# tomvanbraeckel/amv-codec-tools

Measured on AMD Instinct MI355X. Metric: AMV frames/sec/GPU (160x120 decode, bit-exact), higher is better.
Workload: dtype int32; 1 GPU; 160x120 AMV decode, 160000-frame synthetic stream per GPU, chunks resident in HBM; parallelism=frame-range x1, frames_per_gpu=160000, stream=seeded synthetic source (BASELINE.md section 4), every frame

## Files before the change

### amv-codec-tools_amd/csrc/amv_block_load.h

```cpp
#pragma once
#include <cstdlib>

#include "amv_kernels.h"
#include "amv_piece_map.h"

namespace amv {

constexpr uint32_t kSegImageBytes = 60u * 128u;
constexpr uint32_t kScatterSwizzleMask = 0x38u;
constexpr uint32_t kScatterFieldShift = 6u;
constexpr uint32_t kScatterAddressMask = 0x11ffeu;

__device__ __forceinline__ void seg_sync() {
    __builtin_amdgcn_fence(__ATOMIC_SEQ_CST, "wavefront");
    __builtin_amdgcn_wave_barrier();
}

__device__ __forceinline__ bool select_frame(const FrameSel& sel, uint32_t n, uint32_t item, uint32_t& f, uint32_t& slot) {
    f = slot = item;
    if (!sel.round) return true;
    const uint32_t p = sel.base + item;
    if (item >= sel.round || p >= (sel.count ? *sel.count : n)) return false;
    f = sel.list ? sel.list[p] : p;
    return true;
}

struct Segment {
    uint32_t f, slot;
    uint32_t m0, cnt, ok, mcu0;
    uint32_t segidx, nsegs;
};
__device__ __forceinline__ Segment segment_of(uint32_t f, uint32_t slot, const uint32_t* __restrict__ nmcu_ok, const FrameGeom& g,
                                              uint32_t nseg, uint32_t my, uint32_t seg) {
    const uint32_t m0 = seg * kSegMcus;
    return {f, slot, m0, min(kSegMcus, g.mcu_cols - m0), nmcu_ok[f], my * g.mcu_cols + m0, my * nseg + seg, g.mcu_rows * nseg};
}
template <bool kRound>
__device__ __forceinline__ bool next_item(const PieceMap& pm, uint32_t& item) {
    if (!kRound) return false;
    seg_sync();
    item += piece_stride(pm);
    return true;
}

__device__ __forceinline__ bool load_segment_blocks(const SyncSinks& in, const Segment& sg, bool dense_only, const FrameGeom& g,
                                                    uint32_t lane, uint8_t* s_img, uint32_t (&c)[32], bool& skip) {
    const uint32_t f = sg.f, slot = sg.slot, segidx = sg.segidx, nsegs = sg.nsegs, mcu0 = sg.mcu0, cnt = sg.cnt, ok = sg.ok;
    const uint32_t nb = cnt * 6u;
    uint32_t rc = 0xffffffffu, r0 = 0u, r1 = 0u;
    if (in.rec != nullptr && !dense_only) {
        const uint32_t* ss = in.seg_start + ((uint64_t)f * (nsegs + 1u) + segidx) * 2u;
        rc = in.rec_count[f];
        r0 = ss[0];
        r1 = ss[3];
    }
    const bool records = rc != 0xffffffffu;
    skip = !records && in.rec != nullptr && !dense_only;
    if (skip) return false;
    int dc_base = 0;
    if (records) {
        const uint32_t ok_blocks = in.ok_in_blocks ? ok : ok * 6u;
        const uint32_t blocks_ok_here = ok_blocks > mcu0 * 6u ? min(nb, ok_blocks - mcu0 * 6u) : 0u;
        if (!blocks_ok_here) r1 = r0;
        struct __attribute__((packed, aligned(4))) Rec4 { uint32_t w[4]; };
        constexpr uint32_t kAhead = 3;
        const uint32_t* rec = in.rec + (uint64_t)in.rec_line[f] * 32u + r0;
        const uint32_t nrec = r1 - r0;
        Rec4 q[kAhead];
#pragma unroll
        for (uint32_t j = 0; j < kAhead; ++j) {
            const uint32_t i = j * 4u * kWave + lane * 4u;
            q[j] = Rec4{{kDummyRecord, kDummyRecord, kDummyRecord, kDummyRecord}};
            if (i < nrec) q[j] = *reinterpret_cast<const Rec4*>(rec + i);
        }
        uint4* img16 = reinterpret_cast<uint4*>(s_img);
        if (nb == 60u) {
            constexpr uint32_t kWhole = 60u * 8u / kWave;
#pragma unroll
            for (uint32_t j = 0; j < kWhole; ++j) img16[j * kWave + lane] = make_uint4(0, 0, 0, 0);
            if (lane < 60u * 8u - kWhole * kWave) img16[kWhole * kWave + lane] = make_uint4(0, 0, 0, 0);
        } else {
            for (uint32_t i = lane; i < nb * 8u; i += kWave) img16[i] = make_uint4(0, 0, 0, 0);
        }
        seg_sync();
        const uint32_t field0 = (mcu0 * 6u - g.blocks) & 63u;
        const uint32_t first6 = (uint32_t)__builtin_amdgcn_readfirstlane((int)((64u - field0) << kScatterFieldShift));
        const uint32_t ok7 = blocks_ok_here << 7;
        const uint32_t spare = kSegImageBytes + lane * 2u;
        for (uint32_t base = 0;;) {
#pragma unroll
            for (uint32_t j = 0; j < kAhead; ++j) {
                if (base + j * 4u * kWave >= nrec) break;
                if (base + (j + 1u) * 4u * kWave > nrec) {
                    const int32_t left = (int32_t)(nrec - base - j * 4u * kWave) - (int32_t)(lane * 4u);
#pragma unroll
                    for (uint32_t e = 0; e < 4u; ++e)
                        if (left <= (int32_t)e) q[j].w[e] = kDummyRecord;
                }
#pragma unroll
                for (uint32_t e = 0; e < 4u; ++e) {
                    const uint32_t w = q[j].w[e];
                    uint32_t t;
                    asm("v_add_lshl_u32 %0, %1, %2, 1" : "=v"(t) : "v"(w ^ ((w >> 3) & kScatterSwizzleMask)), "s"(first6));
                    const uint32_t at = t & kScatterAddressMask;
                    *reinterpret_cast<int16_t*>(s_img + (at < ok7 ? at : spare)) = (int16_t)(w >> 16);
                }
            }
            base += kAhead * 4u * kWave;
            if (base >= nrec) break;
#pragma unroll
            for (uint32_t j = 0; j < kAhead; ++j) {
                const uint32_t i = base + j * 4u * kWave + lane * 4u;
                if (i < nrec) q[j] = *reinterpret_cast<const Rec4*>(rec + i);
            }
        }
        const uint32_t frame_lanes = ((rc >> 24) & 63u) + 1u;
        if (frame_lanes > 1u) {
            const uint32_t babs = mcu0 * 6u + lane, k6 = lane % 6u;
            const uint4 ent = lane < frame_lanes ? reinterpret_cast<const uint4*>(in.lane_tab)[(uint64_t)f * in.lanes + lane]
                                                 : make_uint4(0xffffffffu, 0u, 0u, 0u);
            uint32_t at = 0u;
#pragma unroll
            for (uint32_t step = 32u; step >= 1u; step >>= 1) {
                const uint32_t probe = at + step;
                const uint32_t first = (uint32_t)__shfl((int)ent.x, (int)(probe & 63u));
                if (probe < frame_lanes && first <= babs) at = probe;
            }
            const int by = __shfl((int)ent.y, (int)at), bu = __shfl((int)ent.z, (int)at), bv = __shfl((int)ent.w, (int)at);
            dc_base = at ? (k6 < 4u ? by : (k6 == 4u ? bu : bv)) : 0;
        }
        seg_sync();
    }
    if (lane >= nb) return false;
    if (records) {
        const uint4* src = reinterpret_cast<const uint4*>(s_img) + lane * 8u;
        const uint32_t swz = (lane + mcu0 * 6u - g.blocks) & 7u;
#pragma unroll
        for (int i = 0; i < 8; ++i) {
            const uint4 q = src[(uint32_t)i ^ swz];
            c[4 * i] = q.x; c[4 * i + 1] = q.y; c[4 * i + 2] = q.z; c[4 * i + 3] = q.w;
        }
        c[0] = (c[0] & 0xffff0000u) | ((c[0] + (uint32_t)dc_base) & 0xffffu);
    } else {
        const uint4* src = reinterpret_cast<const uint4*>(in.coef + (((uint64_t)slot * g.mcus + mcu0) * 6u + lane) * 64u);
#pragma unroll
        for (int i = 0; i < 8; ++i) {
            const uint4 q = src[i];
            c[4 * i] = q.x; c[4 * i + 1] = q.y; c[4 * i + 2] = q.z; c[4 * i + 3] = q.w;
        }
    }
    return true;
}

__device__ __forceinline__ int coef_at(const uint32_t (&c)[32], int i) {
    return (i & 1) ? ((int)c[i >> 1] >> 16) : (int)(int16_t)(c[i >> 1] & 0xffffu);
}

template <class Kernel, class... Tail>
static inline void launch_segments(Kernel part, Kernel walk, uint32_t block, uint32_t row_groups, const SyncSinks& sinks, const uint32_t* nmcu_ok,
                            uint32_t n, const FrameSel& sel, uint32_t items, const FrameGeom& g, hipStream_t s, Tail... tail) {
    for_each_launch(row_groups, segs_per_row(g), items, sel.round != 0u, [&](const PieceMap& pm, uint32_t grid) {
        hipLaunchKernelGGL(sel.round ? walk : part, dim3(grid), dim3(block), 0, s, sinks, nmcu_ok, n, sel, g, pm, tail...);
    });
}

}
```

### amv-codec-tools_amd/csrc/amv_piece_map.h

```cpp
#pragma once
#include <cstdint>
#include <cstdlib>

#include "amv_segment.h"

namespace amv {

struct PieceMap {
    uint32_t row_groups, magic_rg;
    uint32_t nseg, magic_8ns;
    uint32_t units;
    uint32_t item_base;
};
AMV_HD inline uint32_t mul_hi(uint32_t a, uint32_t b) { return (uint32_t)(((uint64_t)a * b) >> 32); }
AMV_HD inline uint32_t div_by(uint32_t b, uint32_t d, uint32_t magic) { return d == 1u ? b : mul_hi(b, magic); }

AMV_HD inline bool locate_piece(const PieceMap& pm, uint32_t b, uint32_t& item0, uint32_t& row_group, uint32_t& seg) {
    const uint32_t octet = pm.nseg == 1u ? b >> 3 : mul_hi(b, pm.magic_8ns);
    const uint32_t within = b - octet * 8u * pm.nseg;
    const uint32_t unit = octet * 8u + (within & 7u);
    seg = within >> 3;
    const uint32_t local = div_by(unit, pm.row_groups, pm.magic_rg);
    row_group = unit - local * pm.row_groups;
    item0 = pm.item_base + local;
    return unit < pm.units;
}
AMV_HD inline uint32_t piece_stride(const PieceMap& pm) { return pm.units / pm.row_groups; }

inline PieceMap make_piece_map(uint32_t row_groups, uint32_t nseg) {
    auto magic = [](uint32_t d) { return (uint32_t)((0x100000000ull + d - 1u) / d); };
    return PieceMap{row_groups, magic(row_groups), nseg, magic(8u * nseg), 0u, 0u};
}
inline uint32_t set_walkers(PieceMap& pm, uint32_t walkers) {
    pm.units = walkers * pm.row_groups;
    return (pm.units + 7u) / 8u * 8u * pm.nseg;
}
inline uint32_t most_items(const PieceMap& pm) {
    const uint32_t widest = 8u * pm.nseg > pm.row_groups ? 8u * pm.nseg : pm.row_groups;
    const uint32_t most = (0xffffffffu / widest - 8u * pm.nseg) / (pm.row_groups * pm.nseg);
    if (const char* e = getenv("AMVHIP_RECON_MOST")) {
        const long v = atol(e);
        if (v > 0 && (unsigned long)v < most) return (uint32_t)v;
    }
    return most;
}

template <class Launch>
static inline void for_each_launch(uint32_t row_groups, uint32_t nseg, uint32_t items, bool round, Launch launch, uint32_t most = 0u) {
    PieceMap pm = make_piece_map(row_groups, nseg);
    if (round) {
        const uint32_t grid = set_walkers(pm, items < kRoundWalkers ? items : kRoundWalkers);
        if (items) launch(pm, grid);
        return;
    }
    if (!most) most = most_items(pm);
    for (uint32_t base = 0; base < items; base += most) {
        pm.item_base = base;
        const uint32_t grid = set_walkers(pm, items - base < most ? items - base : most);
        launch(pm, grid);
    }
}

}
```

### amv-codec-tools_amd/csrc/amv_reconstruct.hip

```cpp
#include "amv_block_load.h"

namespace amv {

namespace {

struct __attribute__((aligned(4))) Px12 { uint32_t w[3]; };

constexpr int kRowsPerGroup = 4;

__device__ __forceinline__ int mad24(int x, int w, int c) {
    int d;
    asm("v_mad_i32_i24 %0, %1, %2, %3" : "=v"(d) : "v"(x), "s"(w), "v"(c));
    return d;
}

enum RowKind { kRowPlain, kRow0, kRow4 };

constexpr uint32_t inverse_of_odd(uint32_t a) {
    uint32_t x = a;
    for (int i = 0; i < 5; ++i) x *= 2u - a * x;
    return x;
}
constexpr int kRowSeed = (int)((64u * inverse_of_odd(181u)) & 0x7fffffffu);
static_assert(181u * 2u * (uint32_t)kRowSeed == 128u, "the seed puts 128 into both 181-products");

template <bool kColumn, RowKind kKind = kRowPlain>
__device__ __forceinline__ void idct8(int& v0, int& v1, int& v2, int& v3, int& v4, int& v5, int& v6, int& v7) {
    constexpr int W1 = 2841, W2 = 2676, W3 = 2408, W5 = 1609, W6 = 1108, W7 = 565;
    constexpr int kBias = kKind == kRow0 ? 128 + 8192 : 128;
    constexpr int kRound = kColumn ? 4 : 0;
    constexpr int kDown = kColumn ? 3 : 0;
    constexpr int kOut = kColumn ? 7 : 8;
    constexpr int kSeed = kColumn ? 0 : kRowSeed, kHalf = kColumn ? 128 : 0;
    int a0 = kColumn ? v0 : v0 * 2048 + kBias, a1 = kColumn ? v4 : v4 * 2048;
    const int i2 = v6, i3 = v2, i4 = v1, i5 = v7, i6 = v5, i7 = v3;
    int t;
    int a4 = mad24(i4, W1, mad24(i5, W7, kRound + kSeed)) >> kDown;
    int a5 = mad24(i4, W7, mad24(i5, -W1, kRound)) >> kDown;
    int a6 = mad24(i6, W5, mad24(i7, W3, kRound - kSeed)) >> kDown;
    int a7 = mad24(i6, W3, mad24(i7, -W5, kRound)) >> kDown;
    t = a0 + a1;
    a0 -= a1;
    int a2 = mad24(i3, W6, mad24(i2, -W2, kRound)) >> kDown;
    int a3 = mad24(i3, W2, mad24(i2, W6, kRound)) >> kDown;
    a1 = a4 + a6;
    a4 -= a6;
    a6 = a5 + a7;
    a5 -= a7;
    a7 = t + a3;
    t -= a3;
    a3 = a0 + a2;
    a0 -= a2;
    a2 = (181 * (a4 + a5) + kHalf) >> 8;
    a4 = (181 * (a4 - a5) + kHalf) >> 8;
    v0 = a7 + a1;
    v1 = a3 + a2;
    v2 = a0 + a4;
    v3 = t + a6;
    v4 = t - a6;
    v5 = a0 - a4;
    v6 = a3 - a2;
    v7 = a7 - a1;
    if (kKind == kRowPlain) {
        v0 >>= kOut; v1 >>= kOut; v2 >>= kOut; v3 >>= kOut; v4 >>= kOut; v5 >>= kOut; v6 >>= kOut; v7 >>= kOut;
    } else {
        v0 &= ~255; v1 &= ~255; v2 &= ~255; v3 &= ~255; v4 &= ~255; v5 &= ~255; v6 &= ~255; v7 &= ~255;
    }
}

struct QuantWords { uint32_t w[2][16]; };
constexpr QuantWords pack_quant() {
    QuantWords q{};
    for (int i = 0; i < 64; ++i) {
        q.w[0][i >> 2] |= (uint32_t)kQuantLuma[i] << (8 * (i & 3));
        q.w[1][i >> 2] |= (uint32_t)kQuantChroma[i] << (8 * (i & 3));
    }
    return q;
}
__device__ const QuantWords kQuantWords = pack_quant();

__device__ __forceinline__ uint32_t clamp_pack(int lo, int hi) {
    uint32_t p, d;
    asm("v_cvt_pk_i16_i32 %0, %1, %2" : "=v"(p) : "v"(lo), "v"(hi));
    asm("v_pk_ashrrev_i16 %0, %1, %2" : "=v"(d) : "s"(0x00070007u), "v"(p));
    return d;
}

constexpr uint32_t pair16(int lo, int hi) { return ((uint32_t)lo & 0xffffu) | ((uint32_t)hi << 16); }
__device__ __forceinline__ uint32_t dot2_bias(uint32_t a, uint32_t w) {
    uint32_t d;
    asm("v_dot2_i32_i16 %0, %1, %2, %3" : "=v"(d) : "v"(a), "s"(w), "v"(32768u));
    return d;
}

struct ChromaTerms { uint32_t bg[2], rb[2], gr[2]; };
__device__ __forceinline__ ChromaTerms chroma_terms(uint32_t uu, uint32_t vv) {
    ChromaTerms c;
#pragma unroll
    for (int e = 0; e < 2; ++e) {
        const uint32_t uv = __builtin_amdgcn_perm(vv, uu, e ? 0x07060302u : 0x05040100u);
        const uint32_t r = dot2_bias(uv, pair16(18, 367));
        const uint32_t gg = dot2_bias(uv, pair16(-159, -220));
        const uint32_t b = dot2_bias(uv, pair16(411, -29));
        c.bg[e] = __builtin_amdgcn_perm(gg, b, 0x06050201u);
        c.rb[e] = __builtin_amdgcn_perm(b, r, 0x06050201u);
        c.gr[e] = __builtin_amdgcn_perm(r, gg, 0x06050201u);
    }
    return c;
}
template <int kLo, int kHi>
__device__ __forceinline__ uint32_t pair_sum(uint32_t yy, uint32_t cc) {
    uint32_t sum;
    if (kLo == 0 && kHi == 0) asm("v_pk_add_i16 %0, %1, %2 op_sel_hi:[0,1]" : "=v"(sum) : "v"(yy), "v"(cc));
    else if (kLo == 0 && kHi == 1) asm("v_pk_add_i16 %0, %1, %2" : "=v"(sum) : "v"(yy), "v"(cc));
    else asm("v_pk_add_i16 %0, %1, %2 op_sel:[1,0]" : "=v"(sum) : "v"(yy), "v"(cc));
    static_assert(kLo <= kHi, "(hi, lo) is not a bracket of the row");
    return sum;
}
__device__ __forceinline__ uint32_t sat_quad(uint32_t lo, uint32_t hi) {
    uint32_t d;
    asm("v_sat_pk_u8_i16 %0, %1" : "=v"(d) : "v"(lo));
    asm("v_sat_pk_u8_i16_sdwa %0, %1 dst_sel:WORD_1 dst_unused:UNUSED_PRESERVE src0_sel:DWORD" : "+v"(d) : "v"(hi));
    return d;
}
__device__ __forceinline__ Px12 patch_row(uint2 yy, const ChromaTerms& c) {
    Px12 v;
    v.w[0] = sat_quad(pair_sum<0, 0>(yy.x, c.bg[0]), pair_sum<0, 1>(yy.x, c.rb[0]));
    v.w[1] = sat_quad(pair_sum<1, 1>(yy.x, c.gr[0]), pair_sum<0, 0>(yy.y, c.bg[1]));
    v.w[2] = sat_quad(pair_sum<0, 1>(yy.y, c.rb[1]), pair_sum<1, 1>(yy.y, c.gr[1]));
    return v;
}

}

template <bool kRound, int kRows>
__global__ __launch_bounds__(kWave * kRows) void amv_reconstruct_kernel(
    SyncSinks in, const uint32_t* __restrict__ nmcu_ok, uint32_t n, FrameSel sel,
    FrameGeom g, PieceMap pm, uint32_t flags, uint8_t* __restrict__ out) {
    constexpr uint32_t kPitchY = kSegMcus * 16, kPitchC = kSegMcus * 8;
    __shared__ __attribute__((aligned(16))) int16_t s_all[kRows][16 * kPitchY + 2 * 8 * kPitchC + 64];
    static_assert((16 * kPitchY + 2 * 8 * kPitchC) * 2 == kSegImageBytes, "the planes reuse the image");
    const uint32_t lane = threadIdx.x & 63u, wave = (uint32_t)__builtin_amdgcn_readfirstlane((int)(threadIdx.x >> 6));
    uint32_t item, row_group, seg;
    if (!locate_piece(pm, blockIdx.x, item, row_group, seg)) return;
    const uint32_t my = row_group * kRows + wave;
    if (my >= g.mcu_rows) return;
    int16_t* const s_mem = s_all[wave];
    int16_t* const s_y = s_mem;
    int16_t* const s_u = s_mem + 16 * kPitchY;
    int16_t* const s_v = s_u + 8 * kPitchC;
    uint8_t* const s_img = reinterpret_cast<uint8_t*>(s_mem);

    uint32_t qw[16];
    {
        const uint4* q4 = reinterpret_cast<const uint4*>(kQuantWords.w[lane % 6u >= 4u ? 1 : 0]);
#pragma unroll
        for (int i = 0; i < 4; ++i) {
            const uint4 q = q4[i];
            qw[4 * i] = q.x; qw[4 * i + 1] = q.y; qw[4 * i + 2] = q.z; qw[4 * i + 3] = q.w;
        }
    }
    do {
    uint32_t f, slot;
    if (!select_frame(sel, n, item, f, slot)) return;
    const Segment sg = segment_of(f, slot, nmcu_ok, g, pm.nseg, my, seg);
    const uint32_t m0 = sg.m0, cnt = sg.cnt, ok = sg.ok, mcu0 = sg.mcu0;

    uint32_t c[32];
    bool skip;
    if (load_segment_blocks(in, sg, kRound, g, lane, s_img, c, skip)) {
        const uint32_t m = lane / 6u, k6 = lane % 6u;
        const bool chroma = k6 >= 4u;
        int v[64];
#pragma unroll
        for (int nat = 0; nat < 64; ++nat) {
            const int scan = kScanOfNatural[nat];
            v[nat] = coef_at(c, scan) * (int)((qw[scan >> 2] >> (8 * (scan & 3))) & 255u);
        }
        if (!(flags & kFlagZigzagFixed))
            v[kAmvlibQuirkNatural] = coef_at(c, kAmvlibQuirkScan) * (int)((qw[kAmvlibQuirkScan >> 2] >> (8 * (kAmvlibQuirkScan & 3))) & 255u);
#pragma unroll
        for (int r = 0; r < 8; ++r) {
            if (r == 0) idct8<false, kRow0>(v[0], v[1], v[2], v[3], v[4], v[5], v[6], v[7]);
            else if (r == 4) idct8<false, kRow4>(v[32], v[33], v[34], v[35], v[36], v[37], v[38], v[39]);
            else idct8<false>(v[8 * r], v[8 * r + 1], v[8 * r + 2], v[8 * r + 3], v[8 * r + 4], v[8 * r + 5], v[8 * r + 6], v[8 * r + 7]);
        }
#pragma unroll
        for (int col = 0; col < 8; ++col)
            idct8<true>(v[col], v[8 + col], v[16 + col], v[24 + col], v[32 + col], v[40 + col], v[48 + col], v[56 + col]);
        int16_t* dst = chroma ? (k6 == 4u ? s_u : s_v) + m * 8u
                              : s_y + ((k6 >> 1) * 8u) * kPitchY + m * 16u + (k6 & 1u) * 8u;
        const uint32_t pitch = chroma ? kPitchC : kPitchY;
#pragma unroll
        for (int r = 0; r < 8; ++r) {
            uint32_t w[4];
#pragma unroll
            for (int q = 0; q < 4; ++q) w[q] = clamp_pack(v[8 * r + 2 * q], v[8 * r + 2 * q + 1]);
            *reinterpret_cast<uint4*>(dst + r * pitch) = make_uint4(w[0], w[1], w[2], w[3]);
        }
    }
    if (skip) return;
    seg_sync();

    const uint32_t vr = min(16u, g.height - my * 16u);
    const uint32_t px = min(cnt * 16u, g.width - m0 * 16u);
    const uint32_t groups = cnt * 4u;
    const bool all_decoded = mcu0 + cnt <= ok;
    uint8_t* const frame = out + (uint64_t)f * g.frame_bytes;
    const uint32_t row0 = (g.height - 1u - my * 16u) * g.stride + m0 * 48u;
    constexpr uint32_t kPairY = 4u * kPitchY, kPairC = 2u * kPitchC, kPlaneU = 32u * kPitchY, kPlaneV = kPlaneU + 16u * kPitchC;
    if (all_decoded && cnt == kSegMcus && px == kSegMcus * 16u && vr == 16u) {
        constexpr uint32_t kGroups = kSegMcus * 4u, kTrips = kGroups * 8u / kWave;
        static_assert(kGroups * 8u % kWave == 0u && kGroups < kWave && kPairC == kGroups * 4u, "whole trips; chroma is linear in t");
        const uint32_t a = lane >= kGroups ? 1u : 0u, b = lane - a * kGroups;
        const uint8_t* const ly = s_img + a * kPairY + b * 8u;
        const uint8_t* const ly_past = ly + (kPairY - kGroups * 8u);
        const uint8_t* const lc = s_img + kPlaneU + lane * 4u;
        const uint32_t off0 = row0 - a * 2u * g.stride + b * 12u;
        const uint32_t off0_past = off0 - 2u * g.stride - kGroups * 12u;
#pragma unroll
        for (uint32_t k = 0; k < kTrips; ++k) {
            const uint32_t q = k * kWave / kGroups, r = k * kWave % kGroups;
            const bool past = r != 0u && b >= kGroups - r;
            const uint8_t* const y = (past ? ly_past : ly) + (q * kPairY + r * 8u);
            const uint2 ya = *reinterpret_cast<const uint2*>(y);
            const uint2 yb = *reinterpret_cast<const uint2*>(y + 2u * kPitchY);
            const uint32_t uu = *reinterpret_cast<const uint32_t*>(lc + k * kWave * 4u);
            const uint32_t vv = *reinterpret_cast<const uint32_t*>(lc + k * kWave * 4u + (kPlaneV - kPlaneU));
            const ChromaTerms c = chroma_terms(uu, vv);
            uint8_t* const upper = frame + (int64_t)(int32_t)(r * 12u - q * 2u * g.stride);
            const uint32_t off = past ? off0_past : off0;
            *reinterpret_cast<Px12*>(upper + off) = patch_row(ya, c);
            *reinterpret_cast<Px12*>(upper - g.stride + off) = patch_row(yb, c);
        }
        continue;
    }
    const uint32_t pairs = (vr + 1u) >> 1;
    const uint32_t step_i2 = kWave / groups, step_gi = kWave - step_i2 * groups;
    uint32_t i2 = lane / groups, gi = lane - i2 * groups;
    for (; i2 < pairs; i2 += step_i2, gi += step_gi) {
        if (gi >= groups) { gi -= groups; ++i2; if (i2 >= pairs) break; }
        const uint32_t lc = gi * 4u;
        uint2 ya = *reinterpret_cast<const uint2*>(s_y + (2u * i2) * kPitchY + lc);
        uint2 yb = *reinterpret_cast<const uint2*>(s_y + (2u * i2 + 1u) * kPitchY + lc);
        uint32_t uu = *reinterpret_cast<const uint32_t*>(s_u + i2 * kPitchC + (lc >> 1));
        uint32_t vv = *reinterpret_cast<const uint32_t*>(s_v + i2 * kPitchC + (lc >> 1));
        if (!all_decoded && (mcu0 + (gi >> 2)) >= ok) {
            constexpr uint32_t kDark = 0xfc00fc00u;
            ya.x = ya.y = yb.x = yb.y = kDark;
            uu = vv = 0u;
        }
        const ChromaTerms c = chroma_terms(uu, vv);
        if (lc >= px) continue;
        uint32_t off = row0 - 2u * i2 * g.stride + lc * 3u;
#pragma unroll
        for (int row = 0; row < 2; ++row) {
            const Px12 v = patch_row(row ? yb : ya, c);
            if (2u * i2 + (uint32_t)row >= vr) break;
            if (lc + 4u <= px) {
                *reinterpret_cast<Px12*>(frame + off) = v;
            } else {
#pragma unroll
                for (uint32_t q = 0; q < 9u; ++q)
                    if (q < (px - lc) * 3u) frame[off + q] = (uint8_t)(v.w[q >> 2] >> (8u * (q & 3u)));
            }
            off -= g.stride;
        }
    }
    } while (next_item<kRound>(pm, item));
}

template <int kRows, class... Args>
static void launch_rows(const FrameGeom& g, Args... args) {
    launch_segments(amv_reconstruct_kernel<false, kRows>, amv_reconstruct_kernel<true, kRows>, kWave * kRows, (g.mcu_rows + kRows - 1) / kRows, args...);
}

void launch_reconstruct(const SyncSinks& sinks, const uint32_t* nmcu_ok, uint32_t n, const FrameSel& sel, uint32_t items,
                        const FrameGeom& g, uint32_t flags, uint8_t* out, hipStream_t s) {
    const uint32_t slots4 = (g.mcu_rows + 3u) / 4u * 4u, slots5 = (g.mcu_rows + 4u) / 5u * 5u;
    const uint32_t waste4 = slots4 - g.mcu_rows, waste5 = slots5 - g.mcu_rows;
    if (10u * waste4 * slots5 >= 10u * waste5 * slots4 + slots4 * slots5) launch_rows<5>(g, sinks, nmcu_ok, n, sel, items, g, s, flags, out);
    else launch_rows<kRowsPerGroup>(g, sinks, nmcu_ok, n, sel, items, g, s, flags, out);
}

__global__ __launch_bounds__(kWave * 4) void amv_expand_records_kernel(SyncSinks in, const uint32_t* __restrict__ nmcu_ok, uint32_t n,
                                                                        FrameGeom g, uint32_t nseg, int16_t* __restrict__ coef) {
    __shared__ __attribute__((aligned(16))) uint8_t s_img[4][kSegImageBytes + 128];
    const uint32_t lane = threadIdx.x & 63u, wave = threadIdx.x >> 6;
    const uint32_t segs = g.mcu_rows * nseg;
    const uint64_t pairs = (uint64_t)n * segs;
    for (uint64_t p = (uint64_t)blockIdx.x * 4u + wave; p < pairs; p += (uint64_t)gridDim.x * 4u) {
        const uint32_t f = (uint32_t)(p / segs), segidx = (uint32_t)(p % segs);
        const Segment sg = segment_of(f, f, nmcu_ok, g, nseg, segidx / nseg, segidx % nseg);
        uint32_t c[32];
        bool skip;
        if (load_segment_blocks(in, sg, false, g, lane, s_img[wave], c, skip)) {
            const uint32_t blk = sg.mcu0 * 6u + lane;
            if (blk >= (in.ok_in_blocks ? sg.ok : sg.ok * 6u)) {
#pragma unroll
                for (int i = 0; i < 32; ++i) c[i] = 0u;
            }
            uint4* d = reinterpret_cast<uint4*>(coef + ((uint64_t)f * g.blocks + blk) * 64u);
#pragma unroll
            for (int i = 0; i < 8; ++i) d[i] = make_uint4(c[4 * i], c[4 * i + 1], c[4 * i + 2], c[4 * i + 3]);
        }
        seg_sync();
    }
}

void launch_expand_records(const SyncSinks& sinks, const uint32_t* nmcu_ok, uint32_t n, const FrameGeom& g, int16_t* coef,
                           hipStream_t s) {
    const uint32_t nseg = segs_per_row(g);
    const uint64_t groups = ((uint64_t)n * g.mcu_rows * nseg + 3u) / 4u;
    if (groups == 0) return;
    hipLaunchKernelGGL(amv_expand_records_kernel, dim3(groups < 65536u ? (uint32_t)groups : 65536u), dim3(kWave * 4), 0, s, sinks,
                       nmcu_ok, n, g, nseg, coef);
}

}
```

Baseline: 31.01 million frames/s.

## Split reconstruct into flat full-row kernel and packed half-row kernel

For 160x120 frames the last MCU row is only 8 pixels tall, so a wave assigned to it left much of its work idle. The reconstruct launch now handles full MCU rows of all frames through a flattened row list, with no per-frame row-group padding. A second kernel packs the short last rows of several frames (a frame and a half per wave) so more lanes carry blocks. The cost is an extra kernel launch and more complex lane-to-block mapping and fallback paths.

```diff
diff --git a/amv-codec-tools_amd/csrc/amv_block_load.h b/amv-codec-tools_amd/csrc/amv_block_load.h
--- a/amv-codec-tools_amd/csrc/amv_block_load.h
+++ b/amv-codec-tools_amd/csrc/amv_block_load.h
@@ -43,8 +43,8 @@
     return true;
 }
 
-__device__ __forceinline__ bool load_segment_blocks(const SyncSinks& in, const Segment& sg, bool dense_only, const FrameGeom& g,
-                                                    uint32_t lane, uint8_t* s_img, uint32_t (&c)[32], bool& skip) {
+__device__ __forceinline__ bool load_segment_blocks_at(const SyncSinks& in, const Segment& sg, bool dense_only, const FrameGeom& g,
+                                                       uint32_t lane, uint32_t blk, uint8_t* s_img, uint32_t (&c)[32], bool& skip) {
     const uint32_t f = sg.f, slot = sg.slot, segidx = sg.segidx, nsegs = sg.nsegs, mcu0 = sg.mcu0, cnt = sg.cnt, ok = sg.ok;
     const uint32_t nb = cnt * 6u;
     uint32_t rc = 0xffffffffu, r0 = 0u, r1 = 0u;
@@ -116,7 +116,7 @@
         }
         const uint32_t frame_lanes = ((rc >> 24) & 63u) + 1u;
         if (frame_lanes > 1u) {
-            const uint32_t babs = mcu0 * 6u + lane, k6 = lane % 6u;
+            const uint32_t babs = mcu0 * 6u + blk, k6 = blk % 6u;
             const uint4 ent = lane < frame_lanes ? reinterpret_cast<const uint4*>(in.lane_tab)[(uint64_t)f * in.lanes + lane]
                                                  : make_uint4(0xffffffffu, 0u, 0u, 0u);
             uint32_t at = 0u;
@@ -131,10 +131,10 @@
         }
         seg_sync();
     }
-    if (lane >= nb) return false;
+    if (blk >= nb) return false;
     if (records) {
-        const uint4* src = reinterpret_cast<const uint4*>(s_img) + lane * 8u;
-        const uint32_t swz = (lane + mcu0 * 6u - g.blocks) & 7u;
+        const uint4* src = reinterpret_cast<const uint4*>(s_img) + blk * 8u;
+        const uint32_t swz = (blk + mcu0 * 6u - g.blocks) & 7u;
 #pragma unroll
         for (int i = 0; i < 8; ++i) {
             const uint4 q = src[(uint32_t)i ^ swz];
@@ -142,7 +142,7 @@
         }
         c[0] = (c[0] & 0xffff0000u) | ((c[0] + (uint32_t)dc_base) & 0xffffu);
     } else {
-        const uint4* src = reinterpret_cast<const uint4*>(in.coef + (((uint64_t)slot * g.mcus + mcu0) * 6u + lane) * 64u);
+        const uint4* src = reinterpret_cast<const uint4*>(in.coef + (((uint64_t)slot * g.mcus + mcu0) * 6u + blk) * 64u);
 #pragma unroll
         for (int i = 0; i < 8; ++i) {
             const uint4 q = src[i];
@@ -150,6 +150,10 @@
         }
     }
     return true;
+}
+__device__ __forceinline__ bool load_segment_blocks(const SyncSinks& in, const Segment& sg, bool dense_only, const FrameGeom& g,
+                                                    uint32_t lane, uint8_t* s_img, uint32_t (&c)[32], bool& skip) {
+    return load_segment_blocks_at(in, sg, dense_only, g, lane, lane, s_img, c, skip);
 }
 
 __device__ __forceinline__ int coef_at(const uint32_t (&c)[32], int i) {
diff --git a/amv-codec-tools_amd/csrc/amv_piece_map.h b/amv-codec-tools_amd/csrc/amv_piece_map.h
--- a/amv-codec-tools_amd/csrc/amv_piece_map.h
+++ b/amv-codec-tools_amd/csrc/amv_piece_map.h
@@ -61,4 +61,56 @@
     }
 }
 
+
+struct RowList {
+    uint32_t rows_full, magic, total;
+};
+inline RowList make_row_list(uint32_t n, uint32_t rows_full) {
+    return RowList{rows_full, rows_full ? (uint32_t)((0x100000000ull + rows_full - 1u) / rows_full) : 0u, n * rows_full};
 }
+AMV_HD inline void flat_row(const RowList& rl, uint32_t r, uint32_t& f, uint32_t& my) {
+    f = div_by(r, rl.rows_full, rl.magic);
+    my = r - f * rl.rows_full;
+}
+
+struct HalfRowPart {
+    uint32_t f, m0, cnt;
+};
+struct HalfRowPlan {
+    uint32_t n, mcu_cols, nseg, magic_ns;
+    uint32_t pack3;
+    uint32_t waves;
+};
+inline HalfRowPlan half_row_plan(uint32_t n, const FrameGeom& g) {
+    HalfRowPlan p;
+    p.n = n;
+    p.mcu_cols = g.mcu_cols;
+    p.nseg = segs_per_row(g);
+    p.magic_ns = (uint32_t)((0x100000000ull + p.nseg - 1u) / p.nseg);
+    p.pack3 = !(g.mcu_cols & 1u) && 6u * g.mcu_cols <= (uint32_t)kWave ? 1u : 0u;
+    p.waves = p.pack3 ? n / 3u * 2u + (n % 3u ? (n % 3u == 1u ? 1u : 2u) : 0u) : n * p.nseg;
+    return p;
+}
+AMV_HD inline void half_row_wave(const HalfRowPlan& p, uint32_t w, HalfRowPart& a, HalfRowPart& b) {
+    if (!p.pack3) {
+        const uint32_t f = div_by(w, p.nseg, p.magic_ns), m0 = (w - f * p.nseg) * kSegMcus;
+        a = HalfRowPart{f, m0, p.mcu_cols - m0 < kSegMcus ? p.mcu_cols - m0 : kSegMcus};
+        b = HalfRowPart{0u, 0u, 0u};
+        return;
+    }
+    const uint32_t f0 = (w >> 1) * 3u, half = p.mcu_cols >> 1;
+    if (!(w & 1u)) {
+        a = HalfRowPart{f0, 0u, p.mcu_cols};
+        b = HalfRowPart{f0 + 1u, 0u, f0 + 1u < p.n ? half : 0u};
+    } else {
+        a = HalfRowPart{f0 + 1u, half, half};
+        b = HalfRowPart{f0 + 2u, 0u, f0 + 2u < p.n ? p.mcu_cols : 0u};
+    }
+}
+inline bool split_rows_ok(uint32_t n, const FrameGeom& g) {
+    const uint32_t last = g.height & 15u, rows_full = g.mcu_rows - 1u, nseg = segs_per_row(g);
+    if (last < 1u || last > 8u || n == 0u) return false;
+    return ((uint64_t)n * rows_full + 4u) * (rows_full ? rows_full : 1u) < 0x100000000ull && ((uint64_t)n * nseg + 4u) * nseg < 0x100000000ull;
+}
+
+}
diff --git a/amv-codec-tools_amd/csrc/amv_reconstruct.hip b/amv-codec-tools_amd/csrc/amv_reconstruct.hip
--- a/amv-codec-tools_amd/csrc/amv_reconstruct.hip
+++ b/amv-codec-tools_amd/csrc/amv_reconstruct.hip
@@ -131,110 +131,40 @@
     return v;
 }
 
-}
-
-template <bool kRound, int kRows>
-__global__ __launch_bounds__(kWave * kRows) void amv_reconstruct_kernel(
-    SyncSinks in, const uint32_t* __restrict__ nmcu_ok, uint32_t n, FrameSel sel,
-    FrameGeom g, PieceMap pm, uint32_t flags, uint8_t* __restrict__ out) {
-    constexpr uint32_t kPitchY = kSegMcus * 16, kPitchC = kSegMcus * 8;
-    __shared__ __attribute__((aligned(16))) int16_t s_all[kRows][16 * kPitchY + 2 * 8 * kPitchC + 64];
-    static_assert((16 * kPitchY + 2 * 8 * kPitchC) * 2 == kSegImageBytes, "the planes reuse the image");
-    const uint32_t lane = threadIdx.x & 63u, wave = (uint32_t)__builtin_amdgcn_readfirstlane((int)(threadIdx.x >> 6));
-    uint32_t item, row_group, seg;
-    if (!locate_piece(pm, blockIdx.x, item, row_group, seg)) return;
-    const uint32_t my = row_group * kRows + wave;
-    if (my >= g.mcu_rows) return;
-    int16_t* const s_mem = s_all[wave];
-    int16_t* const s_y = s_mem;
-    int16_t* const s_u = s_mem + 16 * kPitchY;
-    int16_t* const s_v = s_u + 8 * kPitchC;
-    uint8_t* const s_img = reinterpret_cast<uint8_t*>(s_mem);
-
-    uint32_t qw[16];
-    {
-        const uint4* q4 = reinterpret_cast<const uint4*>(kQuantWords.w[lane % 6u >= 4u ? 1 : 0]);
-#pragma unroll
-        for (int i = 0; i < 4; ++i) {
-            const uint4 q = q4[i];
-            qw[4 * i] = q.x; qw[4 * i + 1] = q.y; qw[4 * i + 2] = q.z; qw[4 * i + 3] = q.w;
-        }
-    }
-    do {
-    uint32_t f, slot;
-    if (!select_frame(sel, n, item, f, slot)) return;
-    const Segment sg = segment_of(f, slot, nmcu_ok, g, pm.nseg, my, seg);
-    const uint32_t m0 = sg.m0, cnt = sg.cnt, ok = sg.ok, mcu0 = sg.mcu0;
-
-    uint32_t c[32];
-    bool skip;
-    if (load_segment_blocks(in, sg, kRound, g, lane, s_img, c, skip)) {
-        const uint32_t m = lane / 6u, k6 = lane % 6u;
-        const bool chroma = k6 >= 4u;
-        int v[64];
-#pragma unroll
-        for (int nat = 0; nat < 64; ++nat) {
-            const int scan = kScanOfNatural[nat];
-            v[nat] = coef_at(c, scan) * (int)((qw[scan >> 2] >> (8 * (scan & 3))) & 255u);
-        }
-        if (!(flags & kFlagZigzagFixed))
-            v[kAmvlibQuirkNatural] = coef_at(c, kAmvlibQuirkScan) * (int)((qw[kAmvlibQuirkScan >> 2] >> (8 * (kAmvlibQuirkScan & 3))) & 255u);
-#pragma unroll
-        for (int r = 0; r < 8; ++r) {
-            if (r == 0) idct8<false, kRow0>(v[0], v[1], v[2], v[3], v[4], v[5], v[6], v[7]);
-            else if (r == 4) idct8<false, kRow4>(v[32], v[33], v[34], v[35], v[36], v[37], v[38], v[39]);
-            else idct8<false>(v[8 * r], v[8 * r + 1], v[8 * r + 2], v[8 * r + 3], v[8 * r + 4], v[8 * r + 5], v[8 * r + 6], v[8 * r + 7]);
-        }
-#pragma unroll
-        for (int col = 0; col < 8; ++col)
-            idct8<true>(v[col], v[8 + col], v[16 + col], v[24 + col], v[32 + col], v[40 + col], v[48 + col], v[56 + col]);
-        int16_t* dst = chroma ? (k6 == 4u ? s_u : s_v) + m * 8u
-                              : s_y + ((k6 >> 1) * 8u) * kPitchY + m * 16u + (k6 & 1u) * 8u;
-        const uint32_t pitch = chroma ? kPitchC : kPitchY;
-#pragma unroll
-        for (int r = 0; r < 8; ++r) {
-            uint32_t w[4];
-#pragma unroll
-            for (int q = 0; q < 4; ++q) w[q] = clamp_pack(v[8 * r + 2 * q], v[8 * r + 2 * q + 1]);
-            *reinterpret_cast<uint4*>(dst + r * pitch) = make_uint4(w[0], w[1], w[2], w[3]);
-        }
-    }
-    if (skip) return;
-    seg_sync();
-
-    const uint32_t vr = min(16u, g.height - my * 16u);
-    const uint32_t px = min(cnt * 16u, g.width - m0 * 16u);
+__device__ __forceinline__ void load_quant(bool chroma, uint32_t (&qw)[16]) {
+    const uint4* q4 = reinterpret_cast<const uint4*>(kQuantWords.w[chroma ? 1 : 0]);
+#pragma unroll
+    for (int i = 0; i < 4; ++i) {
+        const uint4 q = q4[i];
+        qw[4 * i] = q.x; qw[4 * i + 1] = q.y; qw[4 * i + 2] = q.z; qw[4 * i + 3] = q.w;
+    }
+}
+
+__device__ __forceinline__ void transform_block(const uint32_t (&c)[32], const uint32_t (&qw)[16], uint32_t flags, int (&v)[64]) {
+#pragma unroll
+    for (int nat = 0; nat < 64; ++nat) {
+        const int scan = kScanOfNatural[nat];
+        v[nat] = coef_at(c, scan) * (int)((qw[scan >> 2] >> (8 * (scan & 3))) & 255u);
+    }
+    if (!(flags & kFlagZigzagFixed))
+        v[kAmvlibQuirkNatural] = coef_at(c, kAmvlibQuirkScan) * (int)((qw[kAmvlibQuirkScan >> 2] >> (8 * (kAmvlibQuirkScan & 3))) & 255u);
+#pragma unroll
+    for (int r = 0; r < 8; ++r) {
+        if (r == 0) idct8<false, kRow0>(v[0], v[1], v[2], v[3], v[4], v[5], v[6], v[7]);
+        else if (r == 4) idct8<false, kRow4>(v[32], v[33], v[34], v[35], v[36], v[37], v[38], v[39]);
+        else idct8<false>(v[8 * r], v[8 * r + 1], v[8 * r + 2], v[8 * r + 3], v[8 * r + 4], v[8 * r + 5], v[8 * r + 6], v[8 * r + 7]);
+    }
+#pragma unroll
+    for (int col = 0; col < 8; ++col)
+        idct8<true>(v[col], v[8 + col], v[16 + col], v[24 + col], v[32 + col], v[40 + col], v[48 + col], v[56 + col]);
+}
+
+template <uint32_t kPitchY, uint32_t kPitchC>
+__device__ __forceinline__ void store_patches(const int16_t* s_y, const int16_t* s_u, const int16_t* s_v, uint32_t lane, uint8_t* frame,
+                                              uint32_t row0, uint32_t stride, uint32_t vr, uint32_t px, uint32_t cnt, uint32_t mcu0,
+                                              uint32_t ok) {
     const uint32_t groups = cnt * 4u;
     const bool all_decoded = mcu0 + cnt <= ok;
-    uint8_t* const frame = out + (uint64_t)f * g.frame_bytes;
-    const uint32_t row0 = (g.height - 1u - my * 16u) * g.stride + m0 * 48u;
-    constexpr uint32_t kPairY = 4u * kPitchY, kPairC = 2u * kPitchC, kPlaneU = 32u * kPitchY, kPlaneV = kPlaneU + 16u * kPitchC;
-    if (all_decoded && cnt == kSegMcus && px == kSegMcus * 16u && vr == 16u) {
-        constexpr uint32_t kGroups = kSegMcus * 4u, kTrips = kGroups * 8u / kWave;
-        static_assert(kGroups * 8u % kWave == 0u && kGroups < kWave && kPairC == kGroups * 4u, "whole trips; chroma is linear in t");
-        const uint32_t a = lane >= kGroups ? 1u : 0u, b = lane - a * kGroups;
-        const uint8_t* const ly = s_img + a * kPairY + b * 8u;
-        const uint8_t* const ly_past = ly + (kPairY - kGroups * 8u);
-        const uint8_t* const lc = s_img + kPlaneU + lane * 4u;
-        const uint32_t off0 = row0 - a * 2u * g.stride + b * 12u;
-        const uint32_t off0_past = off0 - 2u * g.stride - kGroups * 12u;
-#pragma unroll
-        for (uint32_t k = 0; k < kTrips; ++k) {
-            const uint32_t q = k * kWave / kGroups, r = k * kWave % kGroups;
-            const bool past = r != 0u && b >= kGroups - r;
-            const uint8_t* const y = (past ? ly_past : ly) + (q * kPairY + r * 8u);
-            const uint2 ya = *reinterpret_cast<const uint2*>(y);
-            const uint2 yb = *reinterpret_cast<const uint2*>(y + 2u * kPitchY);
-            const uint32_t uu = *reinterpret_cast<const uint32_t*>(lc + k * kWave * 4u);
-            const uint32_t vv = *reinterpret_cast<const uint32_t*>(lc + k * kWave * 4u + (kPlaneV - kPlaneU));
-            const ChromaTerms c = chroma_terms(uu, vv);
-            uint8_t* const upper = frame + (int64_t)(int32_t)(r * 12u - q * 2u * g.stride);
-            const uint32_t off = past ? off0_past : off0;
-            *reinterpret_cast<Px12*>(upper + off) = patch_row(ya, c);
-            *reinterpret_cast<Px12*>(upper - g.stride + off) = patch_row(yb, c);
-        }
-        continue;
-    }
     const uint32_t pairs = (vr + 1u) >> 1;
     const uint32_t step_i2 = kWave / groups, step_gi = kWave - step_i2 * groups;
     uint32_t i2 = lane / groups, gi = lane - i2 * groups;
@@ -252,7 +182,7 @@
         }
         const ChromaTerms c = chroma_terms(uu, vv);
         if (lc >= px) continue;
-        uint32_t off = row0 - 2u * i2 * g.stride + lc * 3u;
+        uint32_t off = row0 - 2u * i2 * stride + lc * 3u;
 #pragma unroll
         for (int row = 0; row < 2; ++row) {
             const Px12 v = patch_row(row ? yb : ya, c);
@@ -264,19 +194,211 @@
                 for (uint32_t q = 0; q < 9u; ++q)
                     if (q < (px - lc) * 3u) frame[off + q] = (uint8_t)(v.w[q >> 2] >> (8u * (q & 3u)));
             }
-            off -= g.stride;
-        }
-    }
+            off -= stride;
+        }
+    }
+}
+
+}
+
+template <bool kRound, int kRows, bool kFlat = false>
+__global__ __launch_bounds__(kWave * kRows) void amv_reconstruct_kernel(
+    SyncSinks in, const uint32_t* __restrict__ nmcu_ok, uint32_t n, FrameSel sel,
+    FrameGeom g, PieceMap pm, uint32_t flags, uint8_t* __restrict__ out, RowList rl) {
+    static_assert(!(kRound && kFlat), "a round takes its frames whole");
+    constexpr uint32_t kPitchY = kSegMcus * 16, kPitchC = kSegMcus * 8;
+    __shared__ __attribute__((aligned(16))) int16_t s_all[kRows][16 * kPitchY + 2 * 8 * kPitchC + 64];
+    static_assert((16 * kPitchY + 2 * 8 * kPitchC) * 2 == kSegImageBytes, "the planes reuse the image");
+    const uint32_t lane = threadIdx.x & 63u, wave = (uint32_t)__builtin_amdgcn_readfirstlane((int)(threadIdx.x >> 6));
+    uint32_t item, row_group, seg;
+    if (!locate_piece(pm, blockIdx.x, item, row_group, seg)) return;
+    uint32_t my = row_group * kRows + wave, flat_f = 0u;
+    if (kFlat) {
+        const uint32_t r = item * kRows + wave;
+        if (r >= rl.total) return;
+        flat_row(rl, r, flat_f, my);
+    } else if (my >= g.mcu_rows) return;
+    int16_t* const s_mem = s_all[wave];
+    int16_t* const s_y = s_mem;
+    int16_t* const s_u = s_mem + 16 * kPitchY;
+    int16_t* const s_v = s_u + 8 * kPitchC;
+    uint8_t* const s_img = reinterpret_cast<uint8_t*>(s_mem);
+
+    uint32_t qw[16];
+    load_quant(lane % 6u >= 4u, qw);
+    do {
+    uint32_t f, slot;
+    if (kFlat) f = slot = flat_f;
+    else if (!select_frame(sel, n, item, f, slot)) return;
+    const Segment sg = segment_of(f, slot, nmcu_ok, g, pm.nseg, my, seg);
+    const uint32_t m0 = sg.m0, cnt = sg.cnt, ok = sg.ok, mcu0 = sg.mcu0;
+
+    uint32_t c[32];
+    bool skip;
+    if (load_segment_blocks(in, sg, kRound, g, lane, s_img, c, skip)) {
+        const uint32_t m = lane / 6u, k6 = lane % 6u;
+        const bool chroma = k6 >= 4u;
+        int v[64];
+        transform_block(c, qw, flags, v);
+        int16_t* dst = chroma ? (k6 == 4u ? s_u : s_v) + m * 8u
+                              : s_y + ((k6 >> 1) * 8u) * kPitchY + m * 16u + (k6 & 1u) * 8u;
+        const uint32_t pitch = chroma ? kPitchC : kPitchY;
+#pragma unroll
+        for (int r = 0; r < 8; ++r) {
+            uint32_t w[4];
+#pragma unroll
+            for (int q = 0; q < 4; ++q) w[q] = clamp_pack(v[8 * r + 2 * q], v[8 * r + 2 * q + 1]);
+            *reinterpret_cast<uint4*>(dst + r * pitch) = make_uint4(w[0], w[1], w[2], w[3]);
+        }
+    }
+    if (skip) return;
+    seg_sync();
+
+    const uint32_t vr = min(16u, g.height - my * 16u);
+    const uint32_t px = min(cnt * 16u, g.width - m0 * 16u);
+    const bool all_decoded = mcu0 + cnt <= ok;
+    uint8_t* const frame = out + (uint64_t)f * g.frame_bytes;
+    const uint32_t row0 = (g.height - 1u - my * 16u) * g.stride + m0 * 48u;
+    constexpr uint32_t kPairY = 4u * kPitchY, kPairC = 2u * kPitchC, kPlaneU = 32u * kPitchY, kPlaneV = kPlaneU + 16u * kPitchC;
+    if (all_decoded && cnt == kSegMcus && px == kSegMcus * 16u && vr == 16u) {
+        constexpr uint32_t kGroups = kSegMcus * 4u, kTrips = kGroups * 8u / kWave;
+        static_assert(kGroups * 8u % kWave == 0u && kGroups < kWave && kPairC == kGroups * 4u, "whole trips; chroma is linear in t");
+        const uint32_t a = lane >= kGroups ? 1u : 0u, b = lane - a * kGroups;
+        const uint8_t* const ly = s_img + a * kPairY + b * 8u;
+        const uint8_t* const ly_past = ly + (kPairY - kGroups * 8u);
+        const uint8_t* const lc = s_img + kPlaneU + lane * 4u;
+        const uint32_t off0 = row0 - a * 2u * g.stride + b * 12u;
+        const uint32_t off0_past = off0 - 2u * g.stride - kGroups * 12u;
+#pragma unroll
+        for (uint32_t k = 0; k < kTrips; ++k) {
+            const uint32_t q = k * kWave / kGroups, r = k * kWave % kGroups;
+            const bool past = r != 0u && b >= kGroups - r;
+            const uint8_t* const y = (past ? ly_past : ly) + (q * kPairY + r * 8u);
+            const uint2 ya = *reinterpret_cast<const uint2*>(y);
+            const uint2 yb = *reinterpret_cast<const uint2*>(y + 2u * kPitchY);
+            const uint32_t uu = *reinterpret_cast<const uint32_t*>(lc + k * kWave * 4u);
+            const uint32_t vv = *reinterpret_cast<const uint32_t*>(lc + k * kWave * 4u + (kPlaneV - kPlaneU));
+            const ChromaTerms c = chroma_terms(uu, vv);
+            uint8_t* const upper = frame + (int64_t)(int32_t)(r * 12u - q * 2u * g.stride);
+            const uint32_t off = past ? off0_past : off0;
+            *reinterpret_cast<Px12*>(upper + off) = patch_row(ya, c);
+            *reinterpret_cast<Px12*>(upper - g.stride + off) = patch_row(yb, c);
+        }
+        continue;
+    }
+    store_patches<kPitchY, kPitchC>(s_y, s_u, s_v, lane, frame, row0, g.stride, vr, px, cnt, mcu0, ok);
     } while (next_item<kRound>(pm, item));
+}
+
+__global__ __launch_bounds__(kWave * kRowsPerGroup) void amv_reconstruct_half_rows_kernel(
+    SyncSinks in, const uint32_t* __restrict__ nmcu_ok, HalfRowPlan hp, FrameGeom g, uint32_t flags, uint8_t* __restrict__ out) {
+    constexpr uint32_t kMcus = 15, kPitchY = kMcus * 16, kPitchC = kMcus * 8;
+    __shared__ __attribute__((aligned(16))) int16_t s_all[kRowsPerGroup][8 * kPitchY + 2 * 8 * kPitchC + 64];
+    static_assert((8 * kPitchY + 2 * 8 * kPitchC) * 2 == kSegImageBytes, "the planes reuse the image");
+    static_assert(kMcus * 4u <= (uint32_t)kWave && kMcus >= kSegMcus + kSegMcus / 2u, "a frame and a half, a lane per block that shows");
+    const uint32_t lane = threadIdx.x & 63u, wave = (uint32_t)__builtin_amdgcn_readfirstlane((int)(threadIdx.x >> 6));
+    const uint32_t w = blockIdx.x * kRowsPerGroup + wave;
+    if (w >= hp.waves) return;
+    HalfRowPart part[2];
+    half_row_wave(hp, w, part[0], part[1]);
+    int16_t* const s_mem = s_all[wave];
+    int16_t* const s_y = s_mem;
+    int16_t* const s_u = s_mem + 8 * kPitchY;
+    int16_t* const s_v = s_u + 8 * kPitchC;
+    uint8_t* const s_img = reinterpret_cast<uint8_t*>(s_mem);
+
+    const uint32_t split = part[0].cnt * 4u;
+    const bool second = lane >= split;
+    const uint32_t j = lane & 3u;
+    const uint32_t blk = ((lane - (second ? split : 0u)) >> 2) * 6u + (j < 2u ? j : j + 2u);
+    const bool chroma = j >= 2u;
+    uint32_t qw[16];
+    load_quant(chroma, qw);
+
+    const uint32_t my = g.mcu_rows - 1u, nseg = hp.nseg;
+    uint32_t okp[2] = {0u, 0u};
+    bool skip[2] = {true, true};
+    uint32_t c[32];
+    bool have = false;
+#pragma unroll
+    for (int p = 0; p < 2; ++p) {
+        if (part[p].cnt == 0u) continue;
+        const uint32_t f = part[p].f, m0 = part[p].m0;
+        okp[p] = nmcu_ok[f];
+        const Segment sg{f, f, m0, part[p].cnt, okp[p], my * g.mcu_cols + m0, my * nseg + m0 / kSegMcus, g.mcu_rows * nseg};
+        if (load_segment_blocks_at(in, sg, false, g, lane, second == (p == 1) ? blk : 0xffffffffu, s_img, c, skip[p])) have = true;
+        seg_sync();
+    }
+    if (have) {
+        int v[64];
+        transform_block(c, qw, flags, v);
+        const uint32_t m = lane >> 2;
+        int16_t* dst = chroma ? (j == 2u ? s_u : s_v) + m * 8u : s_y + m * 16u + j * 8u;
+        const uint32_t pitch = chroma ? kPitchC : kPitchY;
+#pragma unroll
+        for (int r = 0; r < 8; ++r) {
+            uint32_t q[4];
+#pragma unroll
+            for (int e = 0; e < 4; ++e) q[e] = clamp_pack(v[8 * r + 2 * e], v[8 * r + 2 * e + 1]);
+            *reinterpret_cast<uint4*>(dst + r * pitch) = make_uint4(q[0], q[1], q[2], q[3]);
+        }
+    }
+    seg_sync();
+    const uint32_t vr = g.height - my * 16u;
+    const uint32_t first = my * g.mcu_cols, row_last = (g.height - 1u - my * 16u) * g.stride;
+    if (!skip[0] && !skip[1] && part[0].cnt + part[1].cnt == kMcus && vr == 8u && g.width == g.mcu_cols * 16u &&
+        first + part[0].m0 + part[0].cnt <= okp[0] && first + part[1].cnt <= okp[1]) {
+        constexpr uint32_t kGroups = kMcus * 4u, kPlaneU = 16u * kPitchY, kPlaneV = kPlaneU + 16u * kPitchC;
+        static_assert(2u * kPitchC == kGroups * 4u && 4u * kGroups == 3u * kWave + 48u, "chroma is linear in t; the last trip has 48 patches");
+        uint8_t* const frame = out + (uint64_t)part[0].f * g.frame_bytes;
+        const uint32_t base0 = row_last + part[0].m0 * 48u, base1 = (uint32_t)g.frame_bytes + row_last - split * 12u;
+#pragma unroll
+        for (uint32_t k = 0; k < 4u; ++k) {
+            if (k == 3u && lane >= 4u * kGroups - 3u * kWave) break;
+            const bool past = lane >= kGroups - 4u * k;
+            const uint32_t gi = lane + 4u * k - (past ? kGroups : 0u), i2 = k + (past ? 1u : 0u);
+            const uint8_t* const y = s_img + i2 * (4u * kPitchY) + gi * 8u;
+            const uint2 ya = *reinterpret_cast<const uint2*>(y);
+            const uint2 yb = *reinterpret_cast<const uint2*>(y + 2u * kPitchY);
+            const uint32_t uu = *reinterpret_cast<const uint32_t*>(s_img + kPlaneU + (lane + k * kWave) * 4u);
+            const uint32_t vv = *reinterpret_cast<const uint32_t*>(s_img + kPlaneV + (lane + k * kWave) * 4u);
+            const ChromaTerms c = chroma_terms(uu, vv);
+            const uint32_t off = (gi >= split ? base1 : base0) + gi * 12u - i2 * 2u * g.stride;
+            *reinterpret_cast<Px12*>(frame + off) = patch_row(ya, c);
+            *reinterpret_cast<Px12*>(frame + off - g.stride) = patch_row(yb, c);
+        }
+        return;
+    }
+#pragma unroll
+    for (int p = 0; p < 2; ++p) {
+        if (skip[p]) continue;
+        const uint32_t m0 = part[p].m0, cnt = part[p].cnt, col = p ? part[0].cnt : 0u;
+        uint8_t* const frame = out + (uint64_t)part[p].f * g.frame_bytes;
+        store_patches<kPitchY, kPitchC>(s_y + col * 16u, s_u + col * 8u, s_v + col * 8u, lane, frame,
+                                        (g.height - 1u - my * 16u) * g.stride + m0 * 48u, g.stride, vr, min(cnt * 16u, g.width - m0 * 16u),
+                                        cnt, my * g.mcu_cols + m0, okp[p]);
+    }
 }
 
 template <int kRows, class... Args>
 static void launch_rows(const FrameGeom& g, Args... args) {
-    launch_segments(amv_reconstruct_kernel<false, kRows>, amv_reconstruct_kernel<true, kRows>, kWave * kRows, (g.mcu_rows + kRows - 1) / kRows, args...);
+    launch_segments(amv_reconstruct_kernel<false, kRows>, amv_reconstruct_kernel<true, kRows>, kWave * kRows, (g.mcu_rows + kRows - 1) / kRows, args...,
+                    RowList{});
 }
 
 void launch_reconstruct(const SyncSinks& sinks, const uint32_t* nmcu_ok, uint32_t n, const FrameSel& sel, uint32_t items,
                         const FrameGeom& g, uint32_t flags, uint8_t* out, hipStream_t s) {
+    if (sinks.rec != nullptr && !sel.round && split_rows_ok(items, g)) {
+        const RowList rl = make_row_list(items, g.mcu_rows - 1u);
+        for_each_launch(1u, segs_per_row(g), (rl.total + kRowsPerGroup - 1u) / kRowsPerGroup, false, [&](const PieceMap& pm, uint32_t grid) {
+            hipLaunchKernelGGL((amv_reconstruct_kernel<false, kRowsPerGroup, true>), dim3(grid), dim3(kWave * kRowsPerGroup), 0, s, sinks, nmcu_ok, n,
+                               sel, g, pm, flags, out, rl);
+        });
+        const HalfRowPlan hp = half_row_plan(items, g);
+        hipLaunchKernelGGL(amv_reconstruct_half_rows_kernel, dim3((hp.waves + kRowsPerGroup - 1u) / kRowsPerGroup), dim3(kWave * kRowsPerGroup), 0, s,
+                           sinks, nmcu_ok, hp, g, flags, out);
+        return;
+    }
     const uint32_t slots4 = (g.mcu_rows + 3u) / 4u * 4u, slots5 = (g.mcu_rows + 4u) / 5u * 5u;
     const uint32_t waste4 = slots4 - g.mcu_rows, waste5 = slots5 - g.mcu_rows;
     if (10u * waste4 * slots5 >= 10u * waste5 * slots4 + slots4 * slots5) launch_rows<5>(g, sinks, nmcu_ok, n, sel, items, g, s, flags, out);
```

Result: no change. 31.86 million frames/s (median of 6 runs) (+2.8%).
